# nadimkanazi/cacto

Measured on AMD Instinct MI355X. Metric: env-steps/sec + critic-updates/sec per node, double_integrator & manipulator, higher is better.
Workload: dtype f32 (MLP, MFMA) / f64 (dynamics)

## Files before the change

cacto_amd/_lib.py:

```python
import ctypes as C
import os
import re

HERE = os.path.dirname(os.path.abspath(__file__))
LIB_PATH = os.environ.get("CACTO_HIP_LIB", os.path.join(HERE, "libcacto_hip.so"))
HEADER = os.path.join(HERE, "..", "include", "cacto_hip.h")

CACTO_DYN_SINGLE_INTEGRATOR, CACTO_DYN_CHAIN, CACTO_DYN_CAR, CACTO_DYN_CAR_PARK = 0, 1, 2, 3
CACTO_REW_PLANAR, CACTO_REW_MANIPULATOR, CACTO_REW_UR5, CACTO_REW_CAR_PARK = 0, 1, 2, 3
CACTO_NET_ACTOR, CACTO_NET_CRITIC = 0, 1
MAX_STATE, MAX_ACTION, MAX_JOINTS, JOINT_COLS = 16, 8, 6, 27


class SysParams(C.Structure):
    _fields_ = [
        ("dyn_kind", C.c_int32), ("reward_kind", C.c_int32), ("nb_state", C.c_int32),
        ("nb_action", C.c_int32), ("nq", C.c_int32), ("nv", C.c_int32), ("normalize", C.c_int32),
        ("n_joints", C.c_int32), ("ee_parent", C.c_int32), ("n_check", C.c_int32),
        ("n_weights", C.c_int32), ("const_dyn", C.c_int32),
        ("dt", C.c_double), ("state_norm", C.c_double * MAX_STATE), ("u_max", C.c_double * MAX_ACTION),
        ("w_b", C.c_double), ("scale", C.c_double), ("offset", C.c_double), ("alpha", C.c_double),
        ("alpha2", C.c_double), ("obs", C.c_double * 18), ("target", C.c_double * 3),
        ("w_running", C.c_double * 8), ("w_terminal", C.c_double * 8), ("L_delta", C.c_double),
        ("tau_delta", C.c_double), ("k_db", C.c_double), ("check_points", C.c_double * 20),
# ... 4 lines not shown
class Nets(C.Structure):
    _fields_ = [
        ("actor_d", C.c_void_p), ("actor_m_d", C.c_void_p), ("actor_v_d", C.c_void_p),
        ("critic_d", C.c_void_p), ("critic_m_d", C.c_void_p), ("critic_v_d", C.c_void_p),
        ("target_d", C.c_void_p), ("step_d", C.c_void_p),
    ]


class UpdateCfg(C.Structure):
    _fields_ = [
        ("w_S", C.c_double), ("tau", C.c_double), ("beta1", C.c_double), ("beta2", C.c_double),
        ("epsilon", C.c_double), ("critic_lr", C.c_double * 5), ("actor_lr", C.c_double * 5),
        ("lr_bounds", C.c_double * 4), ("MC", C.c_int32), ("B_global", C.c_int32),
        ("want_target_V", C.c_int32), ("pad", C.c_int32),
    ]


class ToCfg(C.Structure):
    _fields_ = [
        ("max_iter", C.c_int32), ("max_ls", C.c_int32), ("gtol", C.c_double), ("armijo", C.c_double),
        ("mu_min", C.c_double), ("mu_up", C.c_double), ("mu_down", C.c_double), ("mu_max", C.c_double),
        ("poll_every", C.c_int32), ("path", C.c_int32),
    ]


class ToPlan(C.Structure):
    _fields_ = [("on_device", C.c_int32), ("block_threads", C.c_int32), ("lds_bytes", C.c_int32),
                ("launches_per_iter", C.c_int32)]


CACTO_TO_CONVERGED, CACTO_TO_MAXITER, CACTO_TO_FAILED = 0, 1, 2
CACTO_TO_PATH_DEFAULT, CACTO_TO_PATH_WAVE = 0, 1

vp, i32, i64, dbl, flt, sz = C.c_void_p, C.c_int32, C.c_int64, C.c_double, C.c_float, C.c_size_t
_SIGS = {
    "cacto_last_error": (C.c_char_p, []),
    "cacto_abi_version": (C.c_int, []),
    "cacto_sys_create": (C.c_int, [C.POINTER(SysParams), vp, C.POINTER(vp)]),
    "cacto_sys_destroy": (C.c_int, [vp]),
    "cacto_sys_set_critic_type": (C.c_int, [vp, C.c_int]),
    "cacto_env_step_batch": (C.c_int, [vp, vp, vp, vp, vp, vp, vp, vp, vp, C.c_int, vp]),
    "cacto_env_ee": (C.c_int, [vp, vp, vp, C.c_int, vp]),
    "cacto_env_step": (C.c_int, [vp, vp, vp, vp, vp, vp, vp, C.c_int, vp]),
    "cacto_env_jacobians": (C.c_int, [vp, vp, vp, C.c_int, vp, vp, vp]),
    "cacto_env_bound_control_cost": (C.c_int, [vp, vp, vp, C.c_int, vp]),
    "cacto_mlp_param_count": (i64, [vp, C.c_int]),
    "cacto_mlp_netbuf_floats": (i64, [vp, C.c_int]),
    "cacto_mlp_pack": (C.c_int, [vp, C.c_int, vp, vp]),
    "cacto_actor_forward": (C.c_int, [vp, vp, vp, vp, C.c_int, vp]),
    "cacto_critic_forward": (C.c_int, [vp, vp, vp, vp, C.c_int, vp]),
    "cacto_critic_input_grad": (C.c_int, [vp, vp, vp, vp, vp, C.c_int, vp]),
    "cacto_workspace_bytes": (sz, [vp, C.c_int]),
    "cacto_critic_grad": (C.c_int, [vp, C.POINTER(Nets), C.POINTER(UpdateCfg), vp, vp, vp, C.c_int, vp, vp,
                                    vp, vp, vp, sz, vp]),
    "cacto_actor_grad": (C.c_int, [vp, C.POINTER(Nets), C.POINTER(UpdateCfg), vp, vp, C.c_int, vp, vp, sz, vp]),
    "cacto_adam_step": (C.c_int, [vp, C.POINTER(Nets), C.POINTER(UpdateCfg), C.c_int, vp, C.c_int, vp]),
    "cacto_soft_update": (C.c_int, [vp, C.POINTER(Nets), flt, vp]),
    "cacto_update": (C.c_int, [vp, C.POINTER(Nets), C.POINTER(UpdateCfg), vp, vp, vp, C.c_int, vp, vp, vp,
                               vp, sz, vp]),
    "cacto_pipeline_status": (C.c_int, [vp, vp]),
    "cacto_pipeline_check": (C.c_int, [vp, vp]),
    "cacto_update_n": (C.c_int, [vp, C.POINTER(Nets), C.POINTER(UpdateCfg), vp, vp, C.c_int, C.c_int, vp, sz, vp]),
    "cacto_update_n_per": (C.c_int, [vp, C.POINTER(Nets), C.POINTER(UpdateCfg), vp, vp, vp, i64, i64, C.c_double, vp,
                                     vp, C.c_double, C.c_double, C.c_double, vp, C.c_int, C.c_int, vp, sz, vp]),
    "cacto_dp_unique_ids": (C.c_int, [vp, C.c_int]),
    "cacto_dp_attach": (C.c_int, [vp, vp, C.c_int, C.c_int]),
    "cacto_dp_detach": (C.c_int, [vp]),
    "cacto_update_n_dp": (C.c_int, [vp, C.POINTER(Nets), C.POINTER(UpdateCfg), vp, vp, C.c_int, C.c_int, vp, sz,
                                    vp]),
    "cacto_update_n_per_dp": (C.c_int, [vp, C.POINTER(Nets), C.POINTER(UpdateCfg), vp, vp, vp, i64, i64, C.c_double,
                                        vp, vp, C.c_double, C.c_double, C.c_double, vp, C.c_int, C.c_int, vp, sz,
                                        vp]),
    "cacto_update_pair_grads": (C.c_int, [vp, C.POINTER(Nets), C.POINTER(UpdateCfg), vp, vp, vp, vp, C.c_int, vp, vp,
                                          vp, vp, sz, vp]),
    "cacto_update_pair_grads_stage": (C.c_int, [vp, C.POINTER(Nets), C.POINTER(UpdateCfg), vp, vp, vp, vp, C.c_int,
                                                vp, vp, vp, vp, sz, C.c_int, vp]),
    "cacto_update_pair_apply": (C.c_int, [vp, C.POINTER(Nets), C.POINTER(UpdateCfg), vp, C.c_int, C.c_int, C.c_int,
                                          vp]),
    "cacto_rollout": (C.c_int, [vp, vp, vp, vp, C.c_int, C.c_int, vp, vp, vp, vp, vp, vp, vp, C.c_int, vp]),
    "cacto_rollout_sched": (C.c_int, [vp, vp, vp, vp, C.c_int, C.c_int, vp, vp, vp, vp, vp, vp, vp, C.c_int,
                                      C.c_int, C.c_int, vp]),
    "cacto_rollout_rewards": (C.c_int, [vp, vp, vp, vp, C.c_int, C.c_int, vp, vp, vp, C.c_int, vp]),
    "cacto_ddp_backward": (C.c_int, [vp, vp, i64, vp, i64, vp, C.c_int, C.c_double, vp, vp]),
    "cacto_to_backward_gains": (C.c_int, [vp, vp, i64, vp, i64, vp, C.c_int, C.c_double, vp, vp, vp, vp, vp]),
    "cacto_to_forward": (C.c_int, [vp, vp, i64, vp, i64, vp, vp, vp, C.c_int, C.c_double, vp, vp, vp, vp]),
    "cacto_to_workspace_bytes": (sz, [vp, C.c_int, i64]),
    "cacto_to_workspace_bytes_cfg": (sz, [vp, C.c_int, i64, C.POINTER(ToCfg)]),
    "cacto_to_solve": (C.c_int, [vp, vp, vp, i64, vp, C.c_int, i64, C.POINTER(ToCfg), vp, vp, vp, vp, vp, vp, vp, sz,
                                 vp]),
    "cacto_to_solve_plan": (C.c_int, [vp, C.POINTER(ToCfg), C.POINTER(ToPlan)]),
    "cacto_buffer_add": (C.c_int, [vp, vp, i64, i64, vp, i64, vp]),
    "cacto_rl_solve_add": (C.c_int, [vp, vp, i64, vp, i64, vp, vp, vp, C.c_int, C.c_int, i64, C.c_int, C.c_int, vp,
                                     i64, i64, vp, vp]),
    "cacto_buffer_gather": (C.c_int, [vp, vp, vp, C.c_int, vp, vp, vp, vp, vp, vp, vp]),
    "cacto_per_init": (C.c_int, [vp, vp, i64, vp]),
    "cacto_per_set_range": (C.c_int, [vp, vp, i64, i64, i64, i64, dbl, vp]),
    "cacto_per_set_range_max": (C.c_int, [vp, vp, i64, i64, i64, i64, vp, dbl, vp]),
    "cacto_per_sample": (C.c_int, [vp, vp, i64, i64, dbl, vp, C.c_int, vp, vp, vp, vp]),
    "cacto_per_shard_stats": (C.c_int, [vp, vp, i64, vp, vp]),
    "cacto_per_sample_global": (C.c_int, [vp, vp, i64, i64, dbl, vp, C.c_int, vp, C.c_int, vp, vp, vp, vp]),
    "cacto_per_update": (C.c_int, [vp, vp, i64, vp, vp, vp, vp, dbl, dbl, dbl, vp, C.c_int, vp]),
    "cacto_per_set_leaves": (C.c_int, [vp, vp, i64, vp, vp, C.c_int, vp]),
    "cacto_per_update_relo": (C.c_int, [vp, vp, i64, vp, vp, vp, vp, vp, dbl, dbl, dbl, vp, vp, vp, C.c_int, vp]),
}


def header_exports():
    with open(HEADER) as f:
        text = f.read()
    text = re.sub(r"/\*.*?\*/", "", text, flags=re.S)
    return sorted(set(re.findall(r"\b(cacto_[a-z0-9_]+)\s*\(", text)))


class _Lib:
    def __init__(self, path=LIB_PATH):
        if not os.path.exists(path):
            raise RuntimeError("libcacto_hip.so not found at %s — build it with `python -m cacto_amd.build` "
                               "(there is no CPU fallback)" % path)
        self.path = path
        self.dll = C.CDLL(path)
        partial = os.environ.get("CACTO_LIB_PARTIAL") == "1"
        for name, (res, args) in _SIGS.items():
            if partial and not hasattr(self.dll, name):
                continue
            fn = getattr(self.dll, name)
            fn.restype = res
            fn.argtypes = args
        if self.dll.cacto_abi_version() != 1:
            raise RuntimeError("libcacto_hip.so ABI mismatch")

    def call(self, name, *args):
        rc = getattr(self.dll, name)(*args)
        if rc != 0:
            msg = self.dll.cacto_last_error().decode(errors="replace")
            raise RuntimeError("%s failed (%d): %s" % (name, rc, msg))
        return rc

    def raw(self, name):
        return getattr(self.dll, name)


_LIB = None


def lib():
    global _LIB
    if _LIB is None:
        _LIB = _Lib()
    return _LIB
```

cacto_amd/csrc/ddp_kernels.hip:

```cpp
#include <cstdlib>
#include "ddp_device.h"

namespace cacto {

template <int NJ>
__global__ void __launch_bounds__(64) k_env_jacobians(const SysDevice* __restrict__ sdp, const double* __restrict__ S,
                                                      const double* __restrict__ U, int B, double* __restrict__ Fx,
                                                      double* __restrict__ Fu) {
  constexpr int N = DdpDims<NJ>::N, M = DdpDims<NJ>::M, ns = Dims<NJ>::NS, na = Dims<NJ>::NA;
  if constexpr (NJ <= 2) {
    const int b = blockIdx.x * blockDim.x + threadIdx.x;
    if (b >= B) return;
    const SysDevice& sd = *sdp;
    double x[N], A[N * N], Bm[N * M];
#pragma unroll
    for (int k = 0; k < N; ++k) x[k] = S[(size_t)b * ns + k];
    if constexpr (NJ > 0) {
      double Mm[M * M], Minv[M * M];
      chain_mass<NJ>(sd, x, Mm);
      small_inverse<M>(Mm, Minv);
      ddp_jacobians<NJ>(sd, x, Minv, A, Bm);
    } else {
      ddp_jacobians<NJ>(sd, x, nullptr, A, Bm);
    }
// ... 99 lines not shown
#pragma unroll
        for (int k = 0; k < N; ++k)
          if (a_nz<NJ>(k, c)) s += Vxx[r * N + k] * A[k * N + c];
        VA[r * N + c] = s;
      }
#pragma unroll
      for (int c = 0; c < M; ++c) {
        double s = 0.0;
#pragma unroll
        for (int k = 0; k < N; ++k)
          if (b_nz<NJ>(k, c)) s += Vxx[r * N + k] * B[k * M + c];
        VB[r * M + c] = s;
      }
    }
#pragma unroll
    for (int r = 0; r < N; ++r) {
#pragma unroll
      for (int c = 0; c < N; ++c) {
        double s = 0.0;
#pragma unroll
        for (int k = 0; k < N; ++k)
          if (a_nz<NJ>(k, r)) s += A[k * N + r] * VA[k * N + c];
        Qxx[r * N + c] = lxx[r * N + c] + s;
      }
#pragma unroll
      for (int c = 0; c < M; ++c) {
        double s = 0.0;
#pragma unroll
        for (int k = 0; k < N; ++k)
          if (a_nz<NJ>(k, r)) s += A[k * N + r] * VB[k * M + c];
        Qxu[r * M + c] = s;
      }
    }
#pragma unroll
    for (int r = 0; r < M; ++r)
#pragma unroll
      for (int c = 0; c < M; ++c) {
        double s = 0.0;
#pragma unroll
        for (int k = 0; k < N; ++k)
          if (b_nz<NJ>(k, r)) s += B[k * M + r] * VB[k * M + c];
        const double um = p.u_max[r];
        const double luu = r == c ? p.scale * (-w_run[6] * (2.0 + p.w_b * 90.0 * pow(u[r] / um, 8.0) / (um * um))) : 0.0;
        Quu[r * M + c] = luu + s + (r == c ? mu : 0.0);
      }
    double Qi[M * M];
    small_inverse<M>(Quu, Qi);
    double Kk[M];
#pragma unroll
    for (int r = 0; r < M; ++r) {
      double s = 0.0;
#pragma unroll
      for (int k = 0; k < M; ++k) s += Qi[r * M + k] * Qu[k];
      Kk[r] = s;
    }
#pragma unroll
    for (int r = 0; r < N; ++r) {
      double s = 0.0;
#pragma unroll
      for (int k = 0; k < M; ++k) s += Qxu[r * M + k] * Kk[k];
      Vx[r] = Qx[r] - s;
    }
#pragma unroll
    for (int r = 0; r < N; ++r) {
      double QK[M];
#pragma unroll
      for (int c = 0; c < M; ++c) {
        double s = 0.0;
#pragma unroll
        for (int k = 0; k < M; ++k) s += Qxu[r * M + k] * Qi[k * M + c];
        QK[c] = s;
      }
#pragma unroll
      for (int c = 0; c < N; ++c) {
        double s = 0.0;
#pragma unroll
        for (int k = 0; k < M; ++k) s += QK[k] * Qxu[c * M + k];
        Vxx[r * N + c] = Qxx[r * N + c] - s;
      }
    }
#pragma unroll
    for (int k = 0; k < N; ++k) Oe[(size_t)i * ns + k] = Vx[k];
    Oe[(size_t)i * ns + N] = 0.0;
  }
}

template <int NJ>
__global__ void __launch_bounds__(64) k_ddp_riccati_wave(const SysDevice* __restrict__ sdp,
                                                         const double* __restrict__ U, int64_t ldU,
                                                         const int32_t* __restrict__ nsteps, int n_ep, double mu,
                                                         const double* __restrict__ ws, int64_t ldS,
                                                         double* __restrict__ dVdx) {
  using RC = DdpRec<NJ>;
  constexpr int N = RC::N, M = RC::M, ns = Dims<NJ>::NS, na = Dims<NJ>::NA;
  __shared__ double sA[N * N], sB[N * M], sLx[N], sLxx[N * N], sVx[N], sVxx[N * N], sU[M];
  __shared__ double sVA[N * N], sVB[N * M], sQx[N], sQu[M], sQxx[N * N], sQxu[N * M], sQuu[M * M], sQi[M * M];
  __shared__ double sK[M], sQK[N * M];
  const int e = blockIdx.x, lane = threadIdx.x;
  const cacto_sys_params& p = sdp->p;
  const double w6 = p.w_running[6];
  const int Te = nsteps[e];
  if (Te < 0) return;
  double* Oe = dVdx + (size_t)e * ldS * ns;
  const double* Ue = U + (size_t)e * ldU * na;
  {
    const double* rec = ws + (size_t)Te * RC::R * n_ep + e;
    for (int k = lane; k < N; k += 64) sVx[k] = rec[(size_t)(RC::LX + k) * n_ep];
    for (int k = lane; k < N * N; k += 64) sVxx[k] = rec[(size_t)(RC::LXX + k) * n_ep];
  }
  __syncthreads();
  for (int k = lane; k <= N; k += 64) Oe[(size_t)Te * ns + k] = k < N ? sVx[k] : 0.0;
  for (int i = Te - 1; i >= 0; --i) {
    const double* rec = ws + (size_t)i * RC::R * n_ep + e;
    for (int k = lane; k < N * N; k += 64) {
      sA[k] = rec[(size_t)(RC::A + k) * n_ep];
      sLxx[k] = rec[(size_t)(RC::LXX + k) * n_ep];
    }
    for (int k = lane; k < N * M; k += 64) sB[k] = rec[(size_t)(RC::B + k) * n_ep];
    for (int k = lane; k < N; k += 64) sLx[k] = rec[(size_t)(RC::LX + k) * n_ep];
    for (int k = lane; k < M; k += 64) sU[k] = Ue[(size_t)i * na + k];
    __syncthreads();
    for (int o = lane; o < N * N + N * M + N + M; o += 64) {
      double s = 0.0;
      if (o < N * N) {
        const int r = o / N, c = o - r * N;
#pragma unroll
        for (int k = 0; k < N; ++k) s += sVxx[r * N + k] * sA[k * N + c];
        sVA[o] = s;
      } else if (o < N * N + N * M) {
        const int q = o - N * N, r = q / M, c = q - r * M;
#pragma unroll
        for (int k = 0; k < N; ++k) s += sVxx[r * N + k] * sB[k * M + c];
        sVB[q] = s;
      } else if (o < N * N + N * M + N) {
        const int r = o - N * N - N * M;
#pragma unroll
        for (int k = 0; k < N; ++k) s += sA[k * N + r] * sVx[k];
        sQx[r] = sLx[r] + s;
      } else {
        const int j = o - N * N - N * M - N;
        const double um = p.u_max[j], u = sU[j];
        const double lu = p.scale * (-w6 * (2.0 * u + p.w_b * 10.0 * pow(u / um, 9.0) / um));
#pragma unroll
        for (int k = 0; k < N; ++k) s += sB[k * M + j] * sVx[k];
        sQu[j] = lu + s;
      }
    }
    __syncthreads();
    for (int o = lane; o < N * N + N * M + M * M; o += 64) {
      double s = 0.0;
      if (o < N * N) {
        const int r = o / N, c = o - r * N;
#pragma unroll
        for (int k = 0; k < N; ++k) s += sA[k * N + r] * sVA[k * N + c];
        sQxx[o] = sLxx[o] + s;
      } else if (o < N * N + N * M) {
        const int q = o - N * N, r = q / M, c = q - r * M;
#pragma unroll
        for (int k = 0; k < N; ++k) s += sA[k * N + r] * sVB[k * M + c];
        sQxu[q] = s;
      } else {
        const int q = o - N * N - N * M, r = q / M, c = q - r * M;
#pragma unroll
        for (int k = 0; k < N; ++k) s += sB[k * M + r] * sVB[k * M + c];
        const double um = p.u_max[r];
        const double luu =
            r == c ? p.scale * (-w6 * (2.0 + p.w_b * 90.0 * pow(sU[r] / um, 8.0) / (um * um))) : 0.0;
        sQuu[q] = luu + s + (r == c ? mu : 0.0);
      }
    }
    __syncthreads();
    if (lane == 0) {
      double a[M * M], inv[M * M];
#pragma unroll
      for (int k = 0; k < M * M; ++k) a[k] = sQuu[k];
      small_inverse<M>(a, inv);
#pragma unroll
      for (int r = 0; r < M; ++r) {
        double s = 0.0;
#pragma unroll
        for (int k = 0; k < M; ++k) s += inv[r * M + k] * sQu[k];
        sK[r] = s;
      }
#pragma unroll
      for (int k = 0; k < M * M; ++k) sQi[k] = inv[k];
    }
    __syncthreads();
    for (int o = lane; o < N + N * M; o += 64) {
      double s = 0.0;
      if (o < N) {
#pragma unroll
        for (int k = 0; k < M; ++k) s += sQxu[o * M + k] * sK[k];
        sVx[o] = sQx[o] - s;
      } else {
        const int q = o - N, r = q / M, c = q - r * M;
#pragma unroll
        for (int k = 0; k < M; ++k) s += sQxu[r * M + k] * sQi[k * M + c];
        sQK[q] = s;
      }
    }
    __syncthreads();
    for (int o = lane; o < N * N; o += 64) {
      const int r = o / N, c = o - r * N;
      double s = 0.0;
#pragma unroll
      for (int k = 0; k < M; ++k) s += sQK[r * M + k] * sQxu[c * M + k];
      sVxx[o] = sQxx[o] - s;
    }
    for (int k = lane; k <= N; k += 64) Oe[(size_t)i * ns + k] = k < N ? sVx[k] : 0.0;
    __syncthreads();
  }
}

}

using namespace cacto;

namespace {
int ddp_workspace(cacto_sys* sys, size_t bytes, double** out) {
  if (bytes > sys->ddp_ws_bytes) {
    if (sys->ddp_ws) CACTO_CHECK_HIP(hipFree(sys->ddp_ws));
    sys->ddp_ws = nullptr;
    sys->ddp_ws_bytes = 0;
    CACTO_CHECK_HIP(hipMalloc(&sys->ddp_ws, bytes));
    sys->ddp_ws_bytes = bytes;
  }
  *out = static_cast<double*>(sys->ddp_ws);
  return CACTO_OK;
}

template <int NJ>
struct LaunchDdp {
  static int run(const cacto_sys* sys, const double* S, int64_t ldS, const double* U, int64_t ldU, const int32_t* n,
                 int n_ep, double mu, double* out, hipStream_t st) {
    if constexpr (!DdpDims<NJ>::ok) {
      set_error("cacto_ddp_backward: supported for the single integrator, car and prismatic chains (double integrator)");
      return CACTO_EUNSUPPORTED;
    } else {
      const int rk = sys->host.p.reward_kind;
      const bool rk_ok = NJ == -2 ? rk == CACTO_REW_CAR_PARK
                                  : NJ > 0 ? (sys->host.p.const_dyn ? rk == CACTO_REW_PLANAR
                                                                   : rk == CACTO_REW_MANIPULATOR || rk == CACTO_REW_UR5)
                                           : rk == CACTO_REW_PLANAR;
      if (!rk_ok || (NJ > 0 && (sys->host.p.const_dyn ? NJ != 2 : NJ == 2))) {
        set_error("cacto_ddp_backward: unsupported (dynamics, reward) combination");
        return CACTO_EUNSUPPORTED;
      }
      if constexpr (NJ > 2 || NJ == -2) {
        using RC = DdpRec<NJ>;
        double* ws = nullptr;
        const int rc = ddp_workspace(const_cast<cacto_sys*>(sys), (size_t)ldS * RC::R * n_ep * sizeof(double), &ws);
        if (rc != CACTO_OK) return rc;
        static const char* split_env = std::getenv("CACTO_DDP_SPLIT");
        const bool split = NJ > 2 && !(split_env && split_env[0] == '0');
        if constexpr (NJ > 2) {
          if (split) {
            using PC = DdpPrim<NJ>;
            double* pw = nullptr;
            const size_t rec_bytes = (size_t)ldS * RC::R * n_ep * sizeof(double);
            const int rc2 = ddp_workspace(const_cast<cacto_sys*>(sys), rec_bytes + (size_t)ldS * PC::R * n_ep * sizeof(double),
                                          &ws);
            if (rc2 != CACTO_OK) return rc2;
            pw = ws + (size_t)ldS * RC::R * n_ep;
            const dim3 g(ceil_div(n_ep, 64), (unsigned)ldS);
            hipLaunchKernelGGL(k_ddp_prim<NJ>, g, dim3(64), 0, st, sys->dev, S, ldS, U, ldU, n, n_ep, ws, pw);
            CACTO_CHECK_HIP(hipGetLastError());
            hipLaunchKernelGGL(k_ddp_lx<NJ>, g, dim3(64), 0, st, sys->dev, S, ldS, n, n_ep, ws);
            CACTO_CHECK_HIP(hipGetLastError());
            hipLaunchKernelGGL(k_ddp_tan<NJ>, dim3(g.x, g.y, 2 * NJ), dim3(64), 0, st, sys->dev, S, ldS, n, n_ep, ws, pw);
          }
        }
        if (!split)
          hipLaunchKernelGGL(k_ddp_derivs<NJ>, dim3(ceil_div(n_ep, 64), (unsigned)ldS), dim3(64), 0, st, sys->dev, S,
                             ldS, U, ldU, n, n_ep, ws);
        CACTO_CHECK_HIP(hipGetLastError());
        hipLaunchKernelGGL(k_ddp_riccati_wave<NJ>, dim3(n_ep), dim3(64), 0, st, sys->dev, U, ldU, n, n_ep, mu, ws,
                           ldS, out);
      } else {
        hipLaunchKernelGGL(k_ddp_backward<NJ>, dim3(ceil_div(n_ep, 64)), dim3(64), 0, st, sys->dev, S, ldS, U, ldU,
                           n, n_ep, mu, out);
      }
      CACTO_CHECK_HIP(hipGetLastError());
      return CACTO_OK;
    }
  }
};
template <int NJ>
struct LaunchJac {
  static int run(const cacto_sys* sys, const double* S, const double* U, int B, double* Fx, double* Fu,
                 hipStream_t st) {
    if constexpr (!DdpDims<NJ>::ok) {
      set_error("cacto_env_jacobians: unsupported dynamics");
      return CACTO_EUNSUPPORTED;
    } else {
      if (NJ == 2 && !sys->host.p.const_dyn) {
        set_error("cacto_env_jacobians: 2-joint chains are instantiated for the prismatic pair (double integrator)");
        return CACTO_EUNSUPPORTED;
      }
      if constexpr (NJ > 2) {
        using RC = DdpRec<NJ>;
        using PC = DdpPrim<NJ>;
        constexpr int ns = Dims<NJ>::NS;
        const size_t rec = (size_t)2 * RC::R * B, pwn = (size_t)PC::R * B, s2 = (size_t)2 * B * ns;
        double* ws = nullptr;
        const int rc = ddp_workspace(const_cast<cacto_sys*>(sys), (rec + pwn + s2 + B) * sizeof(double), &ws);
        if (rc != CACTO_OK) return rc;
        double* pw = ws + rec;
        double* S2 = pw + pwn;
        int32_t* n1 = reinterpret_cast<int32_t*>(S2 + s2);
        hipLaunchKernelGGL(k_jac_prep<NJ>, dim3(ceil_div(B * 2 * ns, 256)), dim3(256), 0, st, S, B, S2, n1);
        CACTO_CHECK_HIP(hipGetLastError());
        const dim3 g(ceil_div(B, 64), 1);
        hipLaunchKernelGGL(k_ddp_prim<NJ>, g, dim3(64), 0, st, sys->dev, S2, (int64_t)2, U, (int64_t)1, n1, B, ws, pw);
        CACTO_CHECK_HIP(hipGetLastError());
        hipLaunchKernelGGL(k_ddp_tan<NJ>, dim3(g.x, 1, 2 * NJ), dim3(64), 0, st, sys->dev, S2, (int64_t)2, n1, B, ws,
                           pw);
        CACTO_CHECK_HIP(hipGetLastError());
        constexpr int per = RC::N * RC::N + RC::N * RC::M;
        hipLaunchKernelGGL(k_jac_extract<NJ>, dim3(ceil_div(B * per, 256)), dim3(256), 0, st, ws, B, Fx, Fu);
      } else {
        hipLaunchKernelGGL(k_env_jacobians<NJ>, dim3(ceil_div(B, 64)), dim3(64), 0, st, sys->dev, S, U, B, Fx, Fu);
      }
      CACTO_CHECK_HIP(hipGetLastError());
      return CACTO_OK;
    }
  }
};
}

int cacto_ddp_workspace(cacto_sys* sys, size_t bytes, double** out) { return ddp_workspace(sys, bytes, out); }

extern "C" int cacto_ddp_backward(const cacto_sys* sys, const double* S_traj_d, int64_t ldS, const double* U_traj_d,
                                  int64_t ldU, const int32_t* nsteps_d, int n_ep, double mu, double* dVdx_d,
                                  void* stream) {
  CACTO_REQUIRE(sys && S_traj_d && U_traj_d && nsteps_d && dVdx_d && n_ep >= 0 && ldS >= 1 && ldU >= 0,
                "cacto_ddp_backward: bad arguments");
  if (n_ep == 0) return CACTO_OK;
  return dispatch_nj<LaunchDdp>(sys->host.p, sys, S_traj_d, ldS, U_traj_d, ldU, nsteps_d, n_ep, mu, dVdx_d,
                                as_stream(stream));
}

extern "C" int cacto_env_jacobians(const cacto_sys* sys, const double* S_d, const double* A_d, int B, double* Fx_d,
                                   double* Fu_d, void* stream) {
  CACTO_REQUIRE(sys && S_d && A_d && Fx_d && Fu_d && B >= 0, "cacto_env_jacobians: bad arguments");
  if (B == 0) return CACTO_OK;
  return dispatch_nj<LaunchJac>(sys->host.p, sys, S_d, A_d, B, Fx_d, Fu_d, as_stream(stream));
}
```

cacto_amd/to.py:

```python
import ctypes as C

import numpy as np
import torch

from . import _lib as L
from .system import DEVICE, dptr, stream

CONVERGED, MAXITER, FAILED = L.CACTO_TO_CONVERGED, L.CACTO_TO_MAXITER, L.CACTO_TO_FAILED

DEFAULT_CFG = dict(max_iter=400, max_ls=10, gtol=1e-4, armijo=1e-4, mu_min=1e-6, mu_up=10.0, mu_down=10.0,
                   mu_max=1e10, poll_every=8, path=0)
PATHS = {"default": L.CACTO_TO_PATH_DEFAULT, "wave": L.CACTO_TO_PATH_WAVE}


def make_cfg(cfg=None):
    vals = dict(DEFAULT_CFG)
    vals.update(cfg or {})
    unknown = set(vals) - set(DEFAULT_CFG)
    if unknown:
        raise ValueError("unknown TO settings: %s" % sorted(unknown))
    if isinstance(vals["path"], str):
        if vals["path"] not in PATHS:
            raise ValueError("unknown TO path %r (one of %s, or 0 / 1)" % (vals["path"], sorted(PATHS)))
        vals["path"] = PATHS[vals["path"]]
# ... 21 lines not shown
                       status=torch.full((E,), -1, dtype=torch.int32, device=DEVICE),
                       iters=torch.zeros(E, dtype=torch.int32, device=DEVICE), J=torch.zeros(E, 2, **f64))
        c = cfg if isinstance(cfg, L.ToCfg) else make_cfg(cfg)
        nbytes = int(L.lib().raw("cacto_to_workspace_bytes_cfg")(self.sys.handle, E, ldS, C.byref(c)))
        ws = getattr(self, "_to_ws", None)
        if ws is None or ws.numel() < nbytes:
            ws = self._to_ws = torch.empty(max(nbytes, 1), dtype=torch.uint8, device=DEVICE)
        L.lib().call("cacto_to_solve", self.sys.handle, dptr(S0, torch.float64), dptr(U_init, torch.float64), ldU,
                     dptr(nsteps, torch.int32), E, ldS, C.byref(c), dptr(out["S"], torch.float64),
                     dptr(out["U"], torch.float64), dptr(out["step_cost"], torch.float64),
                     dptr(out["status"], torch.int32), dptr(out["iters"], torch.int32), dptr(out["J"], torch.float64),
                     dptr(ws), nbytes, stream())
        return out

    def solve_plan(self, cfg=None):
        c = cfg if isinstance(cfg, L.ToCfg) else make_cfg(cfg)
        plan = L.ToPlan()
        L.lib().call("cacto_to_solve_plan", self.sys.handle, C.byref(c), C.byref(plan))
        return {name: int(getattr(plan, name)) for name, _ in L.ToPlan._fields_}

    def backward_gains_batch(self, S_traj, U_traj, nsteps, mu=0.0):
        E, ldS, ldU = S_traj.shape[0], S_traj.shape[1], U_traj.shape[1]
        ns, na = self.conf.nb_state, self.conf.nb_action
        f64 = dict(dtype=torch.float64, device=DEVICE)
        out = dict(k=torch.zeros(E, ldU, na, **f64), K=torch.zeros(E, ldU, na, ns - 1, **f64),
                   dJ=torch.zeros(E, 3, **f64), pd=torch.full((E,), -1, dtype=torch.int32, device=DEVICE))
        L.lib().call("cacto_to_backward_gains", self.sys.handle, dptr(S_traj, torch.float64), ldS,
                     dptr(U_traj, torch.float64), ldU, dptr(nsteps, torch.int32), E, float(mu), dptr(out["k"]),
                     dptr(out["K"]), dptr(out["dJ"]), dptr(out["pd"]), stream())
        return out

    def forward_batch(self, S_traj, U_traj, k, K, nsteps, alpha=1.0):
        E, ldS, ldU = S_traj.shape[0], S_traj.shape[1], U_traj.shape[1]
        S_new, U_new = torch.zeros_like(S_traj), torch.zeros_like(U_traj)
        cost = torch.zeros(E, ldS, dtype=torch.float64, device=DEVICE)
        L.lib().call("cacto_to_forward", self.sys.handle, dptr(S_traj, torch.float64), ldS,
                     dptr(U_traj, torch.float64), ldU, dptr(k, torch.float64), dptr(K, torch.float64),
                     dptr(nsteps, torch.int32), E, float(alpha), dptr(S_new), dptr(U_new), dptr(cost), stream())
        return S_new, U_new, cost

    def TO_System_Solve(self, ICS_state, init_TO_states, init_TO_controls, T, cfg=None, accept_maxiter=False):
        ns, na = self.conf.nb_state, self.conf.nb_action
        T = int(T)
        S0 = torch.as_tensor(np.asarray(ICS_state, dtype=np.float64).reshape(1, ns), device=DEVICE)
        U = np.zeros((1, max(T, 1), na))
        U[0, :T] = np.asarray(init_TO_controls, dtype=np.float64).reshape(-1, na)[:T]
        out = self.solve_batch(S0, torch.as_tensor(U, device=DEVICE),
                               torch.tensor([T], dtype=torch.int32, device=DEVICE), cfg=cfg)
        status = int(out["status"][0].item())
        states = out["S"][0, :T + 1]
        TO_states = states[:, :ns - 1].cpu().numpy()
        TO_controls = out["U"][0, :T].cpu().numpy()
        if not (status == CONVERGED or (accept_maxiter and status == MAXITER)):
            return 0, TO_controls, TO_states, None, None, None
        EE = torch.empty(T + 1, 3, dtype=torch.float64, device=DEVICE)
        L.lib().call("cacto_env_ee", self.sys.handle, dptr(states.contiguous()), dptr(EE), T + 1, stream())
        return (1, TO_controls, TO_states, EE.cpu().numpy(), float(out["J"][0, 1].item()),
                out["step_cost"][0, :T + 1].cpu().numpy())

    def TO_Solve(self, ICS_state, init_TO_states, init_TO_controls, T, cfg=None, accept_maxiter=False):
        flag, U, X, ee, _, step_cost = self.TO_System_Solve(ICS_state, init_TO_states, init_TO_controls, T, cfg=cfg,
                                                            accept_maxiter=accept_maxiter)
        if flag == 0:
            return None, None, flag, None, None, None
        T = int(T)
        if self.w_S != 0:
            dVdx = self.backward_pass(T + 1, X, U)
        else:
            dVdx = np.zeros((T + 1, self.conf.nb_state))
        t0 = float(np.asarray(ICS_state, dtype=np.float64).reshape(-1)[-1])
        X = np.concatenate((X, t0 + np.transpose(self.conf.dt * np.array([range(T + 1)]))), axis=1)
        return U, X, flag, ee, step_cost, dVdx

    def backward_pass(self, T, TO_states, TO_controls, mu=1e-9):
        ns, na = self.conf.nb_state, self.conf.nb_action
        S = np.zeros((1, T, ns))
        S[0, :, :ns - 1] = np.asarray(TO_states, dtype=np.float64)[:T, :ns - 1]
        U = np.zeros((1, max(T - 1, 1), na))
        U[0, :T - 1] = np.asarray(TO_controls, dtype=np.float64)[:T - 1, :na]
        out = self.backward_pass_batch(torch.as_tensor(S, device=DEVICE), torch.as_tensor(U, device=DEVICE),
                                       torch.tensor([T - 1], dtype=torch.int32, device=DEVICE), mu=mu)
        return out[0].cpu().numpy()

    def backward_pass_batch(self, S_traj, U_traj, nsteps, mu=1e-9, out=None, status=None):
        E, ldS = S_traj.shape[0], S_traj.shape[1]
        if out is None:
            out = torch.zeros_like(S_traj)
        if status is not None:
            nsteps = torch.where(status.to(device=DEVICE) == 0, nsteps.to(device=DEVICE, dtype=torch.int32),
                                 torch.full_like(nsteps, -1, dtype=torch.int32, device=DEVICE)).contiguous()
        L.lib().call("cacto_ddp_backward", self.sys.handle, dptr(S_traj, torch.float64), ldS,
                     dptr(U_traj, torch.float64), U_traj.shape[1], dptr(nsteps, torch.int32), E, float(mu),
                     dptr(out, torch.float64), stream())
        return out
```

include/cacto_hip.h:

```cpp
#ifndef CACTO_HIP_H
#define CACTO_HIP_H

#include <stddef.h>
#include <stdint.h>

#ifdef __cplusplus
extern "C" {
#endif

#define CACTO_ABI_VERSION 1

#define CACTO_OK 0
#define CACTO_EINVAL -1
#define CACTO_EHIP -2
#define CACTO_ENOMEM -3
#define CACTO_EUNSUPPORTED -4

#define CACTO_DYN_SINGLE_INTEGRATOR 0
#define CACTO_DYN_CHAIN 1
#define CACTO_DYN_CAR 2
#define CACTO_DYN_CAR_PARK 3

#define CACTO_REW_PLANAR 0
#define CACTO_REW_MANIPULATOR 1
// ... 88 lines not shown
  double lr_bounds[4];
  int32_t MC;
  int32_t B_global;
  int32_t want_target_V;
  int32_t pad;
} cacto_update_cfg;


size_t cacto_workspace_bytes(const cacto_sys* sys, int B);

int cacto_critic_grad(const cacto_sys* sys, const cacto_nets* nets, const cacto_update_cfg* cfg,
                      const double* storage_d, const int32_t* idx_d, const float* is_w_d, int B,
                      float* grad_d, float* y_d, float* V_d, float* Vt_d,
                      void* workspace_d, size_t workspace_bytes, void* stream);

int cacto_actor_grad(const cacto_sys* sys, const cacto_nets* nets, const cacto_update_cfg* cfg,
                     const double* storage_d, const int32_t* idx_d, int B, float* grad_d,
                     void* workspace_d, size_t workspace_bytes, void* stream);

int cacto_adam_step(const cacto_sys* sys, const cacto_nets* nets, const cacto_update_cfg* cfg, int which,
                    const float* grad_d, int soft_update, void* stream);

int cacto_soft_update(const cacto_sys* sys, const cacto_nets* nets, float tau, void* stream);

int cacto_update(const cacto_sys* sys, const cacto_nets* nets, const cacto_update_cfg* cfg,
                 const double* storage_d, const int32_t* idx_d, const float* is_w_d, int B,
                 float* y_d, float* V_d, float* Vt_d, void* workspace_d, size_t workspace_bytes,
                 void* stream);

int cacto_pipeline_status(const cacto_sys* sys, unsigned long long* out4_h);
int cacto_pipeline_check(cacto_sys* sys, void* stream);
int cacto_update_n(const cacto_sys* sys, const cacto_nets* nets, const cacto_update_cfg* cfg,
                   const double* storage_d, const int32_t* idx_d, int K, int B, void* workspace_d,
                   size_t workspace_bytes, void* stream);

int cacto_update_n_per(const cacto_sys* sys, const cacto_nets* nets, const cacto_update_cfg* cfg,
                       const double* storage_d, double* sum_tree_d, double* min_tree_d, int64_t capacity,
                       int64_t max_idx, double beta, const double* uniforms_d, double* exp_counter_d,
                       double fresh_factor, double eps, double alpha, double* max_priority_d, int K, int B,
                       void* workspace_d, size_t workspace_bytes, void* stream);

int cacto_update_pair_grads(const cacto_sys* sys, const cacto_nets* nets, const cacto_update_cfg* cfg,
                            const double* storage_d, const int32_t* idx_c_d, const float* is_w_d,
                            const int32_t* idx_a_d, int B, float* grad_d, float* y_d, float* V_d,
                            void* workspace_d, size_t workspace_bytes, void* stream);
int cacto_update_pair_grads_stage(const cacto_sys* sys, const cacto_nets* nets, const cacto_update_cfg* cfg,
                                  const double* storage_d, const int32_t* idx_c_d, const float* is_w_d,
                                  const int32_t* idx_a_d, int B, float* grad_d, float* y_d, float* V_d,
                                  void* workspace_d, size_t workspace_bytes, int stage, void* stream);
int cacto_update_pair_apply(const cacto_sys* sys, const cacto_nets* nets, const cacto_update_cfg* cfg,
                            const float* grad_d, int critic, int actor, int soft_update, void* stream);

int cacto_dp_unique_ids(void* out_h, int n);
int cacto_dp_attach(cacto_sys* sys, const void* ids_h, int rank, int world);
int cacto_dp_detach(cacto_sys* sys);
int cacto_update_n_dp(const cacto_sys* sys, const cacto_nets* nets, const cacto_update_cfg* cfg,
                      const double* storage_d, const int32_t* idx_d, int K, int B, void* workspace_d,
                      size_t workspace_bytes, void* stream);
int cacto_update_n_per_dp(const cacto_sys* sys, const cacto_nets* nets, const cacto_update_cfg* cfg,
                          const double* storage_d, double* sum_tree_d, double* min_tree_d, int64_t capacity,
                          int64_t max_idx, double beta, const double* uniforms_d, double* exp_counter_d,
                          double fresh_factor, double eps, double alpha, double* max_priority_d, int K, int B,
                          void* workspace_d, size_t workspace_bytes, void* stream);


int cacto_rollout(const cacto_sys* sys, const float* actor_netbuf_d, const double* S0_d,
                  const int32_t* nsteps_d, int T, int use_actor, const double* W_d,
                  double* S_traj_d, float* A_traj_d, double* R_traj_d, double* EE_traj_d,
                  int32_t* status_d, const int32_t* order_d, int B, void* stream);

int cacto_rollout_sched(const cacto_sys* sys, const float* actor_netbuf_d, const double* S0_d,
                        const int32_t* nsteps_d, int T, int use_actor, const double* W_d,
                        double* S_traj_d, float* A_traj_d, double* R_traj_d, double* EE_traj_d,
                        int32_t* status_d, const int32_t* order_d, int B, int groups, int workgroups,
                        void* stream);

int cacto_rollout_rewards(const cacto_sys* sys, const double* S_traj_d, const float* A_traj_d,
                          const int32_t* nsteps_d, int T, int use_actor, const double* W_d,
                          double* R_traj_d, double* EE_traj_d, int B, void* stream);

int cacto_ddp_backward(const cacto_sys* sys, const double* S_traj_d, int64_t ldS, const double* U_traj_d,
                       int64_t ldU, const int32_t* nsteps_d, int n_ep, double mu, double* dVdx_d, void* stream);



enum cacto_to_status {
  CACTO_TO_CONVERGED = 0,
  CACTO_TO_MAXITER = 1,
  CACTO_TO_FAILED = 2
};

typedef struct {
  int32_t max_iter;
  int32_t max_ls;
  double gtol;
  double armijo;
  double mu_min, mu_up, mu_down, mu_max;
  int32_t poll_every;
  int32_t path;
} cacto_to_cfg;

enum cacto_to_path {
  CACTO_TO_PATH_DEFAULT = 0,
  CACTO_TO_PATH_WAVE = 1
};

int cacto_to_backward_gains(const cacto_sys* sys, const double* S_d, int64_t ldS, const double* U_d, int64_t ldU,
                            const int32_t* nsteps_d, int n_ep, double mu, double* k_d, double* K_d, double* dJ_d,
                            int32_t* pd_d, void* stream);

int cacto_to_forward(const cacto_sys* sys, const double* S_d, int64_t ldS, const double* U_d, int64_t ldU,
                     const double* k_d, const double* K_d, const int32_t* nsteps_d, int n_ep, double alpha,
                     double* S_new_d, double* U_new_d, double* cost_new_d, void* stream);

size_t cacto_to_workspace_bytes(const cacto_sys* sys, int n_ep, int64_t ldS);
size_t cacto_to_workspace_bytes_cfg(const cacto_sys* sys, int n_ep, int64_t ldS, const cacto_to_cfg* cfg_h);

int cacto_to_solve(const cacto_sys* sys, const double* S0_d, const double* U_init_d, int64_t ldU,
                   const int32_t* nsteps_d, int n_ep, int64_t ldS, const cacto_to_cfg* cfg_h, double* S_d,
                   double* U_d, double* step_cost_d, int32_t* status_d, int32_t* iters_d, double* J_d, void* ws_d,
                   size_t ws_bytes, void* stream);

typedef struct {
  int32_t on_device;
  int32_t block_threads;
  int32_t lds_bytes;
  int32_t launches_per_iter;
} cacto_to_plan;

int cacto_to_solve_plan(const cacto_sys* sys, const cacto_to_cfg* cfg_h, cacto_to_plan* out);


int cacto_buffer_add(const cacto_sys* sys, double* storage_d, int64_t capacity, int64_t next_idx,
                     const double* rows_d, int64_t n, void* stream);

int cacto_rl_solve_add(const cacto_sys* sys, const double* S_traj_d, int64_t ldS, const double* R_d,
                       int64_t ldR, const double* R_term_d, const double* dVdx_d, const int64_t* row_off_d,
                       int n_ep, int max_T, int64_t total_rows, int nsteps_td, int mc, double* storage_d,
                       int64_t capacity, int64_t next_idx, double* total_d, void* stream);

int cacto_buffer_gather(const cacto_sys* sys, const double* storage_d, const int32_t* idx_d, int B,
                        float* S_d, float* R_d, float* S_next_d, float* dVdx_d, float* d_d, double* term_d,
                        void* stream);

int cacto_per_init(double* sum_tree_d, double* min_tree_d, int64_t capacity, void* stream);
int cacto_per_set_range(double* sum_tree_d, double* min_tree_d, int64_t capacity, int64_t ring_size,
                        int64_t start, int64_t n, double value, void* stream);
int cacto_per_set_range_max(double* sum_tree_d, double* min_tree_d, int64_t capacity, int64_t ring_size,
                            int64_t start, int64_t n, const double* max_priority_d, double alpha, void* stream);
int cacto_per_sample(const double* sum_tree_d, const double* min_tree_d, int64_t capacity, int64_t max_idx,
                     double beta, const double* uniforms_d, int B, int32_t* idx_d, float* is_w_d,
                     double* exp_counter_d, void* stream);
int cacto_per_shard_stats(const double* sum_tree_d, const double* min_tree_d, int64_t max_idx, double* stats_d,
                          void* stream);
int cacto_per_sample_global(const double* sum_tree_d, const double* min_tree_d, int64_t capacity, int64_t max_idx,
                            double beta, const double* uniforms_d, int B, const double* shard_stats_d,
                            int n_shards, int32_t* idx_d, float* is_w_d, double* exp_counter_d, void* stream);
int cacto_per_update(double* sum_tree_d, double* min_tree_d, int64_t capacity, const int32_t* idx_d,
                     const float* y_d, const float* V_d, const double* exp_counter_d, double fresh_factor,
                     double eps, double alpha, double* max_priority_d, int B, void* stream);
int cacto_per_update_relo(double* sum_tree_d, double* min_tree_d, int64_t capacity, const int32_t* idx_d,
                          const float* y_d, const float* V_d, const float* Vt_d, const double* exp_counter_d,
                          double fresh_factor, double eps, double alpha, double* max_priority_d, double* leaves_ws_d,
                          int32_t* status_d, int B, void* stream);
int cacto_per_set_leaves(double* sum_tree_d, double* min_tree_d, int64_t capacity, const int32_t* idx_d,
                         const double* values_d, int n, void* stream);
// ... 6 lines not shown
```

Measured before the change: 692.8 million.

## Parallelize DDP backward Riccati recursion across lane groups per episode

Adds a new DDP backward kernel that gives each episode a group of G lanes (default 16). The lanes compute the per-step cost derivatives for G timesteps in parallel, then split the Riccati dot products (Q terms and the value update) across lanes through LDS with wavefront barriers. The goal is to replace the old one-thread-per-episode serial recursion, which had few active threads and long dependency chains when there are few episodes. The previous kernel is kept as a reference entry point. In exchange, the new kernel adds many wave-level syncs and LDS traffic per timestep and runs fewer episodes per wavefront.

```diff
diff --git a/cacto_amd/_lib.py b/cacto_amd/_lib.py
--- a/cacto_amd/_lib.py
+++ b/cacto_amd/_lib.py
@@ -110,6 +110,7 @@
                                       C.c_int, C.c_int, vp]),
     "cacto_rollout_rewards": (C.c_int, [vp, vp, vp, vp, C.c_int, C.c_int, vp, vp, vp, C.c_int, vp]),
     "cacto_ddp_backward": (C.c_int, [vp, vp, i64, vp, i64, vp, C.c_int, C.c_double, vp, vp]),
+    "cacto_ddp_backward_ref": (C.c_int, [vp, vp, i64, vp, i64, vp, C.c_int, C.c_double, vp, vp]),
     "cacto_to_backward_gains": (C.c_int, [vp, vp, i64, vp, i64, vp, C.c_int, C.c_double, vp, vp, vp, vp, vp]),
     "cacto_to_forward": (C.c_int, [vp, vp, i64, vp, i64, vp, vp, vp, C.c_int, C.c_double, vp, vp, vp, vp]),
     "cacto_to_workspace_bytes": (sz, [vp, C.c_int, i64]),
diff --git a/cacto_amd/csrc/ddp_kernels.hip b/cacto_amd/csrc/ddp_kernels.hip
--- a/cacto_amd/csrc/ddp_kernels.hip
+++ b/cacto_amd/csrc/ddp_kernels.hip
@@ -205,6 +205,281 @@
 #pragma unroll
     for (int k = 0; k < N; ++k) Oe[(size_t)i * ns + k] = Vx[k];
     Oe[(size_t)i * ns + N] = 0.0;
+  }
+}
+
+#ifndef CACTO_DDP_LANES_G
+#define CACTO_DDP_LANES_G 16
+#endif
+
+template <int NJ>
+struct DdpLane {
+  static constexpr int N = DdpDims<NJ>::N, M = DdpDims<NJ>::M;
+  static constexpr bool AB_STEP = NJ == -1;
+  static constexpr int LX = 0, LXX = LX + N, LU = LXX + N * N, LUU = LU + M, RA = LUU + M, RB = RA + N * N,
+                       R = (AB_STEP ? RB + N * M : RA) | 1;
+  static constexpr int CA = 0, CB = CA + N * N, VX = CB + N * M, VXX = VX + N, VA = VXX + N * N, VB = VA + N * N,
+                       QX = VB + N * M, QU = QX + N, QXX = QU + M, QXU = QXX + N * N, QUU = QXU + N * M,
+                       W = QUU + M * M;
+};
+
+__device__ __forceinline__ void ddp_lane_sync() {
+  __builtin_amdgcn_fence(__ATOMIC_ACQ_REL, "wavefront");
+  __builtin_amdgcn_wave_barrier();
+}
+
+struct DdpDot {
+  int x, xs, y, ys, l, out;
+  unsigned nz;
+  bool xr, yr, ld_l, add_l, add_mu, mu_nz, valid;
+};
+
+template <int NJ, int PHASE>
+__device__ __forceinline__ DdpDot ddp_lane_dot(int o, int so) {
+  using LC = DdpLane<NJ>;
+  constexpr int N = LC::N, M = LC::M;
+  const int a = LC::AB_STEP ? LC::RA : so + LC::CA, b = LC::AB_STEP ? LC::RB : so + LC::CB;
+  DdpDot d{0, 0, 0, 0, 0, 0, 0u, false, false, false, false, false, false, false};
+  unsigned am[N], bm[M];
+#pragma unroll
+  for (int c = 0; c < N; ++c) {
+    am[c] = 0u;
+#pragma unroll
+    for (int k = 0; k < N; ++k) am[c] |= a_nz<NJ>(k, c) ? 1u << k : 0u;
+  }
+#pragma unroll
+  for (int c = 0; c < M; ++c) {
+    bm[c] = 0u;
+#pragma unroll
+    for (int k = 0; k < N; ++k) bm[c] |= b_nz<NJ>(k, c) ? 1u << k : 0u;
+  }
+  auto pick = [](const unsigned* m, int n, int c) {
+    unsigned v = 0u;
+#pragma unroll
+    for (int i = 0; i < n; ++i) v = c == i ? m[i] : v;
+    return v;
+  };
+  if constexpr (PHASE == 1) {
+    if (o < N * N) {
+      const int r = o / N, c = o - r * N;
+      d.x = so + LC::VXX + r * N, d.xs = 1, d.y = a + c, d.ys = N, d.yr = LC::AB_STEP;
+      d.nz = pick(am, N, c), d.out = so + LC::VA + o, d.valid = true;
+    } else if (o < N * N + N * M) {
+      const int q = o - N * N, r = q / M, c = q - r * M;
+      d.x = so + LC::VXX + r * N, d.xs = 1, d.y = b + c, d.ys = M, d.yr = LC::AB_STEP;
+      d.nz = pick(bm, M, c), d.out = so + LC::VB + q, d.valid = true;
+    } else if (o < N * N + N * M + N) {
+      const int r = o - N * N - N * M;
+      d.x = a + r, d.xs = N, d.xr = LC::AB_STEP, d.y = so + LC::VX, d.ys = 1;
+      d.nz = pick(am, N, r), d.l = LC::LX + r, d.ld_l = d.add_l = true, d.out = so + LC::QX + r, d.valid = true;
+    } else if (o < N * N + N * M + N + M) {
+      const int c = o - N * N - N * M - N;
+      d.x = b + c, d.xs = M, d.xr = LC::AB_STEP, d.y = so + LC::VX, d.ys = 1;
+      d.nz = pick(bm, M, c), d.l = LC::LU + c, d.ld_l = d.add_l = true, d.out = so + LC::QU + c, d.valid = true;
+    }
+  } else {
+    if (o < N * N) {
+      const int r = o / N, c = o - r * N;
+      d.x = a + r, d.xs = N, d.xr = LC::AB_STEP, d.y = so + LC::VA + c, d.ys = N;
+      d.nz = pick(am, N, r), d.l = LC::LXX + o, d.ld_l = d.add_l = true, d.out = so + LC::QXX + o, d.valid = true;
+    } else if (o < N * N + N * M) {
+      const int q = o - N * N, r = q / M, c = q - r * M;
+      d.x = a + r, d.xs = N, d.xr = LC::AB_STEP, d.y = so + LC::VB + c, d.ys = M;
+      d.nz = pick(am, N, r), d.out = so + LC::QXU + q, d.valid = true;
+    } else if (o < N * N + N * M + M * M) {
+      const int q = o - N * N - N * M, r = q / M, c = q - r * M;
+      d.x = b + r, d.xs = M, d.xr = LC::AB_STEP, d.y = so + LC::VB + c, d.ys = M;
+      d.nz = pick(bm, M, r), d.l = LC::LUU + r, d.ld_l = d.mu_nz = r == c, d.add_l = d.add_mu = true;
+      d.out = so + LC::QUU + q, d.valid = true;
+    }
+  }
+  return d;
+}
+
+template <int N>
+__device__ __forceinline__ void ddp_lane_eval(const DdpDot& d, double* base, int ro, double mu) {
+  const double* x = base + d.x + (d.xr ? ro : 0);
+  const double* y = base + d.y + (d.yr ? ro : 0);
+  double xv[N], yv[N];
+#pragma unroll
+  for (int k = 0; k < N; ++k) {
+    xv[k] = x[k * d.xs];
+    yv[k] = y[k * d.ys];
+  }
+  const double lr = base[ro + d.l];
+  const double lv = d.ld_l ? lr : 0.0;
+  double s = 0.0;
+#pragma unroll
+  for (int k = 0; k < N; ++k) {
+    const double t = xv[k] * yv[k];
+    s = (d.nz >> k & 1u) ? s + t : s;
+  }
+  double v = d.add_l ? lv + s : s;
+  v = d.add_mu ? v + (d.mu_nz ? mu : 0.0) : v;
+  if (d.valid) base[d.out] = v;
+}
+
+template <int NJ, int G>
+__global__ void __launch_bounds__(64) k_ddp_backward_lanes(const SysDevice* __restrict__ sdp,
+                                                           const double* __restrict__ S, int64_t ldS,
+                                                           const double* __restrict__ U, int64_t ldU,
+                                                           const int32_t* __restrict__ nsteps, int n_ep, double mu,
+                                                           double* __restrict__ dVdx) {
+  using LC = DdpLane<NJ>;
+  constexpr int N = DdpDims<NJ>::N, M = DdpDims<NJ>::M, ns = Dims<NJ>::NS, na = Dims<NJ>::NA;
+  constexpr int EPW = 64 / G, GS = G * LC::R + LC::W;
+  static_assert(G == 8 || G == 16 || G == 32, "lane groups of 8, 16 or 32");
+  __shared__ double lds[EPW * GS];
+  const int lane = threadIdx.x, g = lane / G, j = lane % G;
+  const int e = blockIdx.x * EPW + g;
+  const SysDevice& sd = *sdp;
+  const cacto_sys_params& p = sd.p;
+  int Te = e < n_ep ? nsteps[e] : -1;
+  if (Te < 0) Te = -1;
+  int Tmax = Te;
+#pragma unroll
+  for (int o = G; o < 64; o *= 2) Tmax = max(Tmax, __shfl_xor(Tmax, o));
+  if (Tmax < 0) return;
+  const size_t eo = Te >= 0 ? e : 0;
+  const double* Se = S + eo * ldS * ns;
+  const double* Ue = U + eo * ldU * na;
+  double* Oe = dVdx + eo * ldS * ns;
+  double* rec = lds + g * GS;
+  double* st = rec + G * LC::R;
+  double w_run[7], w_term[7];
+#pragma unroll
+  for (int k = 0; k < 7; ++k) {
+    w_run[k] = p.w_running[k];
+    w_term[k] = p.w_terminal[k];
+  }
+  if (Te >= 0 && j == 0) {
+    double x[N], Vx[N], Vxx[N * N];
+#pragma unroll
+    for (int k = 0; k < N; ++k) x[k] = Se[(size_t)Te * ns + k];
+    ddp_lx<NJ>(sd, w_term, x, Vx, Vxx);
+#pragma unroll
+    for (int k = 0; k < N; ++k) {
+      st[LC::VX + k] = Vx[k];
+      Oe[(size_t)Te * ns + k] = Vx[k];
+    }
+    Oe[(size_t)Te * ns + N] = 0.0;
+#pragma unroll
+    for (int k = 0; k < N * N; ++k) st[LC::VXX + k] = Vxx[k];
+    if constexpr (!LC::AB_STEP) {
+      double Minv[NJ > 0 ? M * M : 1], A[N * N], B[N * M];
+      if constexpr (NJ > 0) {
+        double Mm[M * M], q[NJ];
+#pragma unroll
+        for (int i = 0; i < NJ; ++i) q[i] = Se[i];
+        chain_mass<NJ>(sd, q, Mm);
+        small_inverse<M>(Mm, Minv);
+      }
+      ddp_jacobians<NJ>(sd, x, Minv, A, B);
+#pragma unroll
+      for (int k = 0; k < N * N; ++k) st[LC::CA + k] = A[k];
+#pragma unroll
+      for (int k = 0; k < N * M; ++k) st[LC::CB + k] = B[k];
+    }
+  }
+  ddp_lane_sync();
+  constexpr int T1 = N * N + N * M + N + M, T2 = N * N + N * M + M * M, T3 = N * N + N;
+  constexpr int NT1 = (T1 + G - 1) / G, NT2 = (T2 + G - 1) / G, NT3 = (T3 + G - 1) / G;
+  DdpDot d1[NT1], d2[NT2];
+#pragma unroll
+  for (int t = 0; t < NT1; ++t) d1[t] = ddp_lane_dot<NJ, 1>(t * G + j, G * LC::R);
+#pragma unroll
+  for (int t = 0; t < NT2; ++t) d2[t] = ddp_lane_dot<NJ, 2>(t * G + j, G * LC::R);
+  const double* sQxu = st + LC::QXU;
+  for (int b0 = 0; b0 < Tmax; b0 += G) {
+    const int i0 = Te - 1 - b0;
+    if (i0 - j >= 0) {
+      const int i = i0 - j;
+      double x[N], u[M], lx[N], lxx[N * N];
+#pragma unroll
+      for (int k = 0; k < N; ++k) x[k] = Se[(size_t)i * ns + k];
+#pragma unroll
+      for (int k = 0; k < M; ++k) u[k] = Ue[(size_t)i * na + k];
+      ddp_lx<NJ>(sd, w_run, x, lx, lxx);
+      double* r = rec + j * LC::R;
+#pragma unroll
+      for (int k = 0; k < N; ++k) r[LC::LX + k] = lx[k];
+#pragma unroll
+      for (int k = 0; k < N * N; ++k) r[LC::LXX + k] = lxx[k];
+#pragma unroll
+      for (int c = 0; c < M; ++c) {
+        const double um = p.u_max[c];
+        r[LC::LU + c] = p.scale * (-w_run[6] * (2.0 * u[c] + p.w_b * 10.0 * pow(u[c] / um, 9.0) / um));
+        r[LC::LUU + c] = p.scale * (-w_run[6] * (2.0 + p.w_b * 90.0 * pow(u[c] / um, 8.0) / (um * um)));
+      }
+      if constexpr (LC::AB_STEP) {
+        double A[N * N], B[N * M];
+        ddp_jacobians<NJ>(sd, x, nullptr, A, B);
+#pragma unroll
+        for (int k = 0; k < N * N; ++k) r[LC::RA + k] = A[k];
+#pragma unroll
+        for (int k = 0; k < N * M; ++k) r[LC::RB + k] = B[k];
+      }
+    }
+    ddp_lane_sync();
+    const int nsub = min(G, Tmax - b0);
+    for (int s0 = 0; s0 < nsub; ++s0) {
+      const int i = i0 - s0;
+      const bool act = i >= 0;
+      const int ro = s0 * LC::R;
+      if (act) {
+#pragma unroll
+        for (int t = 0; t < NT1; ++t) ddp_lane_eval<N>(d1[t], rec, ro, mu);
+      }
+      ddp_lane_sync();
+      if (act) {
+#pragma unroll
+        for (int t = 0; t < NT2; ++t) ddp_lane_eval<N>(d2[t], rec, ro, mu);
+      }
+      ddp_lane_sync();
+      if (act) {
+        double Quu[M * M], Qi[M * M], Kk[M];
+#pragma unroll
+        for (int k = 0; k < M * M; ++k) Quu[k] = st[LC::QUU + k];
+        small_inverse<M>(Quu, Qi);
+#pragma unroll
+        for (int r = 0; r < M; ++r) {
+          double s = 0.0;
+#pragma unroll
+          for (int k = 0; k < M; ++k) s += Qi[r * M + k] * st[LC::QU + k];
+          Kk[r] = s;
+        }
+#pragma unroll
+        for (int t = 0; t < NT3; ++t) {
+          const int o = t * G + j;
+          const bool vx = o >= N * N, valid = o < T3;
+          const int r = !valid ? 0 : vx ? o - N * N : o / N, c = vx || !valid ? r : o - r * N;
+          double qr[M], qc[M], QK[M];
+#pragma unroll
+          for (int k = 0; k < M; ++k) {
+            qr[k] = sQxu[r * M + k];
+            qc[k] = sQxu[c * M + k];
+          }
+          const double q = st[!valid ? 0 : vx ? LC::QX + r : LC::QXX + o];
+#pragma unroll
+          for (int cc = 0; cc < M; ++cc) {
+            double s = 0.0;
+#pragma unroll
+            for (int k = 0; k < M; ++k) s += qr[k] * Qi[k * M + cc];
+            QK[cc] = s;
+          }
+          double s = 0.0;
+#pragma unroll
+          for (int k = 0; k < M; ++k) s += (vx ? qr[k] : QK[k]) * (vx ? Kk[k] : qc[k]);
+          const double v = q - s;
+          if (valid) st[vx ? LC::VX + r : LC::VXX + o] = v;
+          if (valid && vx) {
+            Oe[(size_t)i * ns + r] = v;
+            if (r == N - 1) Oe[(size_t)i * ns + N] = 0.0;
+          }
+        }
+      }
+      ddp_lane_sync();
+    }
   }
 }
 
@@ -355,7 +630,7 @@
 template <int NJ>
 struct LaunchDdp {
   static int run(const cacto_sys* sys, const double* S, int64_t ldS, const double* U, int64_t ldU, const int32_t* n,
-                 int n_ep, double mu, double* out, hipStream_t st) {
+                 int n_ep, double mu, double* out, hipStream_t st, bool ref) {
     if constexpr (!DdpDims<NJ>::ok) {
       set_error("cacto_ddp_backward: supported for the single integrator, car and prismatic chains (double integrator)");
       return CACTO_EUNSUPPORTED;
@@ -399,9 +674,13 @@
         CACTO_CHECK_HIP(hipGetLastError());
         hipLaunchKernelGGL(k_ddp_riccati_wave<NJ>, dim3(n_ep), dim3(64), 0, st, sys->dev, U, ldU, n, n_ep, mu, ws,
                            ldS, out);
-      } else {
+      } else if (ref) {
         hipLaunchKernelGGL(k_ddp_backward<NJ>, dim3(ceil_div(n_ep, 64)), dim3(64), 0, st, sys->dev, S, ldS, U, ldU,
                            n, n_ep, mu, out);
+      } else {
+        constexpr int G = CACTO_DDP_LANES_G;
+        hipLaunchKernelGGL((k_ddp_backward_lanes<NJ, G>), dim3(ceil_div(n_ep, 64 / G)), dim3(64), 0, st, sys->dev, S,
+                           ldS, U, ldU, n, n_ep, mu, out);
       }
       CACTO_CHECK_HIP(hipGetLastError());
       return CACTO_OK;
@@ -460,7 +739,17 @@
                 "cacto_ddp_backward: bad arguments");
   if (n_ep == 0) return CACTO_OK;
   return dispatch_nj<LaunchDdp>(sys->host.p, sys, S_traj_d, ldS, U_traj_d, ldU, nsteps_d, n_ep, mu, dVdx_d,
-                                as_stream(stream));
+                                as_stream(stream), false);
+}
+
+extern "C" int cacto_ddp_backward_ref(const cacto_sys* sys, const double* S_traj_d, int64_t ldS,
+                                      const double* U_traj_d, int64_t ldU, const int32_t* nsteps_d, int n_ep,
+                                      double mu, double* dVdx_d, void* stream) {
+  CACTO_REQUIRE(sys && S_traj_d && U_traj_d && nsteps_d && dVdx_d && n_ep >= 0 && ldS >= 1 && ldU >= 0,
+                "cacto_ddp_backward_ref: bad arguments");
+  if (n_ep == 0) return CACTO_OK;
+  return dispatch_nj<LaunchDdp>(sys->host.p, sys, S_traj_d, ldS, U_traj_d, ldU, nsteps_d, n_ep, mu, dVdx_d,
+                                as_stream(stream), true);
 }
 
 extern "C" int cacto_env_jacobians(const cacto_sys* sys, const double* S_d, const double* A_d, int B, double* Fx_d,
diff --git a/cacto_amd/to.py b/cacto_amd/to.py
--- a/cacto_amd/to.py
+++ b/cacto_amd/to.py
@@ -127,14 +127,15 @@
                                        torch.tensor([T - 1], dtype=torch.int32, device=DEVICE), mu=mu)
         return out[0].cpu().numpy()
 
-    def backward_pass_batch(self, S_traj, U_traj, nsteps, mu=1e-9, out=None, status=None):
+    def backward_pass_batch(self, S_traj, U_traj, nsteps, mu=1e-9, out=None, status=None, ref=False):
         E, ldS = S_traj.shape[0], S_traj.shape[1]
         if out is None:
             out = torch.zeros_like(S_traj)
         if status is not None:
             nsteps = torch.where(status.to(device=DEVICE) == 0, nsteps.to(device=DEVICE, dtype=torch.int32),
                                  torch.full_like(nsteps, -1, dtype=torch.int32, device=DEVICE)).contiguous()
-        L.lib().call("cacto_ddp_backward", self.sys.handle, dptr(S_traj, torch.float64), ldS,
+        L.lib().call("cacto_ddp_backward_ref" if ref else "cacto_ddp_backward", self.sys.handle,
+                     dptr(S_traj, torch.float64), ldS,
                      dptr(U_traj, torch.float64), U_traj.shape[1], dptr(nsteps, torch.int32), E, float(mu),
                      dptr(out, torch.float64), stream())
         return out
diff --git a/include/cacto_hip.h b/include/cacto_hip.h
--- a/include/cacto_hip.h
+++ b/include/cacto_hip.h
@@ -194,6 +194,9 @@
 int cacto_ddp_backward(const cacto_sys* sys, const double* S_traj_d, int64_t ldS, const double* U_traj_d,
                        int64_t ldU, const int32_t* nsteps_d, int n_ep, double mu, double* dVdx_d, void* stream);
 
+int cacto_ddp_backward_ref(const cacto_sys* sys, const double* S_traj_d, int64_t ldS, const double* U_traj_d,
+                           int64_t ldU, const int32_t* nsteps_d, int n_ep, double mu, double* dVdx_d, void* stream);
+
 
 
 enum cacto_to_status {
```

New measurement: 692.6 million. No clear change (-0.0%).
